# roseDwayane/EyeGaze-Multimodal

Measured on AMD Instinct MI355X. Metric: train samples/sec (gaze+EEG windows), higher is better.
Workload: dtype bf16; 1 GPU; cfg3: BASELINE configs[2]/[3]: + bidirectional cross-stream attention fusion; batch_per_gpu=256, global_batch=256, C=8, T=1024, seq_len=65, d_model=256, layers=6, step=fwd(train,dropout)+bwd+allreduce+clip+AdamW, parallelism=dp1

## Files before the change

### eyegaze_multimodal_amd/csrc/ffn.hip

```cpp
#include <type_traits>
#include "lnproj.h"

namespace {

constexpr int FR = RT_ROWS;
constexpr int FD = RT_COLS;
constexpr int FC = 128;
constexpr int F_XT = RT_TILEB;
constexpr int F_HT = FR * FC * 2;
constexpr int F_LDS = F_XT + 2 * F_HT;

template <typename T>
struct FfnArgs {
  const T* A; const T* W1; const T* W2; T* H; T* C; const float* bias1; const float* bias2; const T* gate; const T* residual;
  const unsigned long long* bits_in; unsigned long long* bits_out;
  const float* ln_gamma; const float* ln_beta; T* LN_OUT; float* ln_stats;
  const eg_step_state* st;
  long long lda, ldh, ldc, ldg, ldr;
  int M, F, relu, res_in_lds;
  DropCfg dh, dc1, dc2;
  float gate_scale;
};

struct FfnNoTail {};
template <typename T, int GATE, int BOUT, int EPI, bool LNF = false, bool KEEP = true, bool TAIL = false>
__global__ __launch_bounds__(256, 2) void ffn_chain_kernel(FfnArgs<T> p, std::conditional_t<TAIL, LnProjArgs<T>, FfnNoTail> q) {
  static_assert(!TAIL || (GATE == 2 && BOUT == 0 && EPI == 0 && !LNF && KEEP), "the norm-1 tail follows the backward form only");
  typedef typename H16<T>::frag frag;
  extern __shared__ __attribute__((aligned(16))) char smem[];
  char* const xt = smem;
  char* const hb = smem + F_XT;
  const int tid = threadIdx.x, lane = tid & 63;
  const int wn = __builtin_amdgcn_readfirstlane(tid >> 6);
  const int l15 = lane & 15, g4 = lane >> 4;
  const int m0 = blockIdx.x * FR;
  const int nch = p.F / FC;

#pragma unroll
  for (int i = 0; i < RT_DMA_PER_WAVE; ++i) {
    const int row = min(m0 + rt_dma_row(wn, lane, i), p.M - 1);
    rt_dma_issue((const char*)(p.A + (size_t)row * (size_t)p.lda), xt, wn, lane, i);
  }

  const char* const w1u = (const char*)(p.W1 + rt_frag_elem<8, 2>(0, wn, 0, 0));
  const char* const w2u = (const char*)(p.W2 + rt_frag_elem<4, 4>(0, wn, 0, 0));
  const uint32_t wl = (uint32_t)lane * 16u;
  frag w1r[4][2], w2r[2][4];
  auto req_w1 = [&](int c, int s, int slot) {
#pragma unroll
    for (int j = 0; j < 2; ++j) w1r[slot][j] = *(const frag*)(w1u + rt_frag_elem<8, 2>(c, 0, s, j) * 2 + wl);
  };
  auto req_w2 = [&](int c, int s, int slot) {
#pragma unroll
    for (int j = 0; j < 4; ++j) w2r[slot][j] = *(const frag*)(w2u + rt_frag_elem<4, 4>(c, 0, s, j) * 2 + wl);
  };
#pragma unroll
  for (int s = 0; s < 4; ++s) req_w1(0, s, s);
#pragma unroll
  for (int s = 0; s < 2; ++s) req_w2(0, s, s);

  f32x4 acc2[5][4];
#pragma unroll
  for (int i = 0; i < 5; ++i)
#pragma unroll
    for (int j = 0; j < 4; ++j) acc2[i][j] = (f32x4){0.f, 0.f, 0.f, 0.f};

  uint32_t seed_lo = 0, seed_hi = 0;
  if (p.dh.thresh | p.dc1.thresh | p.dc2.thresh) { seed_lo = p.st->seed_lo; seed_hi = p.st->seed_hi; }

  uint32_t touched = 0;
  if (wn < 2) {
    const char* wb = (const char*)(wn == 0 ? p.W1 : p.W2);
    const int lines = p.F * FD * 2 / 128;
    const int per = (lines + gridDim.x - 1) / gridDim.x;
    for (int t = lane; t < per; t += 64) {
      const int g = blockIdx.x * per + t;
      if (g < lines) touched += *(const uint32_t*)(wb + (size_t)g * 128);
    }
  }
  asm volatile("s_waitcnt vmcnt(0)" ::: "memory");
  asm volatile("" :: "v"(touched));
  __syncthreads();

  const unsigned long long* const bits_p = p.bits_in ? p.bits_in + ((size_t)blockIdx.x * nch * 4 + wn) * 64 + lane : nullptr;
  unsigned long long gnext0 = 0, gnext1 = 0;
  if (GATE == 2) {
    gnext0 = bits_p[0];
    if (nch > 1) gnext1 = bits_p[256];
  }
  const int rbase = l15;
  const int sw7 = rt_swz(l15);
  int ha[2];
#pragma unroll
  for (int j = 0; j < 2; ++j) {
    const int hcol = 32 * wn + 16 * j + 4 * g4;
    ha[j] = l15 * 256 + (((hcol >> 3) ^ sw7) << 4) + ((hcol & 4) << 1);
  }
  const uint32_t pair0 = ((uint32_t)(m0 + l15) * (uint32_t)p.F + (uint32_t)(32 * wn + 4 * g4)) >> 1;
  const uint32_t pairF = 8u * (uint32_t)p.F;

  for (int c = 0; c < nch; ++c) {
    char* const hc = hb + (c & 1) * F_HT;
    const int f0 = FC * c + 32 * wn + 4 * g4;

    float b1[2][4];
#pragma unroll
    for (int j = 0; j < 2; ++j) {
#pragma unroll
      for (int q = 0; q < 4; ++q) b1[j][q] = 0.f;
      if (EPI == 3 || (EPI == 4 && p.bias1)) load4(p.bias1 + f0 + 16 * j, b1[j]);
    }

    u32x2 gt[5][2];
    if (GATE == 1) {
      int rb = rbase;
      asm volatile("" : "+v"(rb));
#pragma unroll
      for (int i = 0; i < 5; ++i) {
        const int m = min(m0 + rb + 16 * i, p.M - 1);
#pragma unroll
        for (int j = 0; j < 2; ++j) gt[i][j] = *(const u32x2*)(p.gate + (size_t)m * (size_t)p.ldg + f0 + 16 * j);
      }
    }
    uint32_t gw[2] = {0u, 0u}, ow[2] = {0u, 0u};
    if (GATE == 2) {
      gw[0] = (uint32_t)gnext0;
      gw[1] = (uint32_t)(gnext0 >> 32);
      gnext0 = gnext1;
      if (c + 2 < nch) gnext1 = bits_p[(size_t)(c + 2) * 256];
    }

    f32x4 acc1[5][2];
#pragma unroll
    for (int i = 0; i < 5; ++i)
#pragma unroll
      for (int j = 0; j < 2; ++j) acc1[i][j] = (f32x4){0.f, 0.f, 0.f, 0.f};
#pragma unroll
    for (int s = 0; s < 8; ++s) {
      frag xf[5];
      rt_frags<T>(xt, rbase, g4, sw7, s, xf);
#pragma unroll
      for (int i = 0; i < 5; ++i)
#pragma unroll
        for (int j = 0; j < 2; ++j) acc1[i][j] = H16<T>::mfma(w1r[s & 3][j], xf[i], acc1[i][j]);
      if (s < 4) req_w1(c, s + 4, s & 3);
      else if (c + 1 < nch) req_w1(c + 1, s - 4, s & 3);
    }

    const uint32_t pairc = pair0 + (uint32_t)(FC / 2) * (uint32_t)c;
#pragma unroll
    for (int i = 0; i < 5; ++i) {
#pragma unroll
      for (int j = 0; j < 2; ++j) {
        const int t = 2 * i + j;
        float v[4];
#pragma unroll
        for (int q = 0; q < 4; ++q) {
          v[q] = acc1[i][j][q];
          if (EPI == 3 || EPI == 4) v[q] += b1[j][q];
          if (EPI == 3) v[q] = fmaxf(v[q], 0.f);
          if (EPI == 4 && p.relu) v[q] = fmaxf(v[q], 0.f);
        }
        if (GATE == 1) {
          float gv[4];
          load4((const T*)&gt[i][j], gv);
#pragma unroll
          for (int q = 0; q < 4; ++q) v[q] = gv[q] > 0.f ? v[q] * p.gate_scale : 0.f;
        }
        if (GATE == 2) {
#pragma unroll
          for (int q = 0; q < 4; ++q) {
            const int n = (2 * t + (q >> 1)) % 10;
            int m;
            asm("v_bfe_i32 %0, %1, %2, 1" : "=v"(m) : "v"(gw[t / 5]), "n"((9 - n) + 16 * (q & 1)));
            v[q] = __uint_as_float(__float_as_uint(v[q] * p.gate_scale) & (uint32_t)m);
          }
        }
        if (p.dh.thresh) {
          const uint32_t e = pairc + (uint32_t)(8 * j) + (uint32_t)i * pairF;
          const uint32_t h0 = eg_hash(seed_lo, seed_hi, p.dh.site, e), h1 = eg_hash(seed_lo, seed_hi, p.dh.site, e + 1u);
          v[0] = (h0 & 0xFFFFu) >= p.dh.thresh ? v[0] * p.dh.scale : 0.0f;
          v[1] = (h0 >> 16) >= p.dh.thresh ? v[1] * p.dh.scale : 0.0f;
          v[2] = (h1 & 0xFFFFu) >= p.dh.thresh ? v[2] * p.dh.scale : 0.0f;
          v[3] = (h1 >> 16) >= p.dh.thresh ? v[3] * p.dh.scale : 0.0f;
        }
        const u32x2 pk = pack4<T>(v);
        *(u32x2*)(hc + ha[j] + 4096 * i) = pk;
        if (BOUT) {
#pragma unroll
          for (int h = 0; h < 2; ++h) {
            uint32_t z, f;
            asm("v_pk_max_i16 %0, %1, 0" : "=v"(z) : "v"(pk[h]));
            asm("v_pk_min_u16 %0, %1, %2" : "=v"(f) : "v"(z), "v"(0x00010001u));
            ow[t / 5] = (ow[t / 5] << 1) | f;
          }
        }
      }
    }
    if (BOUT) p.bits_out[((size_t)blockIdx.x * nch + c) * 256 + wn * 64 + lane] = (unsigned long long)ow[0] | ((unsigned long long)ow[1] << 32);
    __syncthreads();

    if constexpr (KEEP) {
      int tq = tid >> 4;
      asm volatile("" : "+v"(tq));
#pragma unroll
      for (int ps = 0; ps < 5; ++ps) {
        const int r = 16 * ps + tq, ch = tid & 15;
        const u32x4 o = *(const u32x4*)(hc + r * 256 + rt_piece(r, ch));
        if (m0 + r < p.M) *(u32x4*)(p.H + (size_t)(m0 + r) * (size_t)p.ldh + FC * c + 8 * ch) = o;
      }
    }

#pragma unroll
    for (int s = 0; s < 4; ++s) {
      frag hf[5];
      rt_frags<T, FC * 2>(hc, rbase, g4, sw7, s, hf);
#pragma unroll
      for (int i = 0; i < 5; ++i)
#pragma unroll
        for (int j = 0; j < 4; ++j) acc2[i][j] = H16<T>::mfma(w2r[s & 1][j], hf[i], acc2[i][j]);
      if (s < 2) req_w2(c, s + 2, s & 1);
      else if (c + 1 < nch) req_w2(c + 1, s - 2, s & 1);
    }
  }
  __syncthreads();

  float* timg = (float*)(hb + wn * RT_IMGB);
  const int er = lane >> 2, ec = lane & 3;
  const int n = 64 * wn + 16 * ec;
  float bv[16];
#pragma unroll
  for (int j = 0; j < 16; ++j) bv[j] = 0.f;
  if (p.bias2) { load8(p.bias2 + n, bv); load8(p.bias2 + n + 8, bv + 8); }
  u32x4 eraw[5][2];
#pragma unroll
  for (int i = 0; i < 5; ++i) {
    eraw[i][0] = (u32x4){0u, 0u, 0u, 0u};
    eraw[i][1] = (u32x4){0u, 0u, 0u, 0u};
    const int r = 16 * i + er;
    if (p.res_in_lds) {
      rt_tile_row16(xt, r, n, eraw[i][0], eraw[i][1]);
    } else if (p.residual && m0 + r < p.M) {
      const T* pe = p.residual + (size_t)(m0 + r) * (size_t)p.ldr + n;
      eraw[i][0] = *(const u32x4*)pe;
      eraw[i][1] = *(const u32x4*)(pe + 8);
    }
  }
  const int tl = lane & 31, thw = tid >> 5;
  u32x4 xr[TAIL ? LP_ROWS_PER_HW : 1];
  float mean[TAIL ? LP_ROWS_PER_HW : 1], rstd[TAIL ? LP_ROWS_PER_HW : 1];
  if constexpr (TAIL) {
#pragma unroll
    for (int j = 0; j < LP_ROWS_PER_HW; ++j) {
      const int m = min(m0 + thw + 8 * j, q.M - 1);
      xr[j] = *(const u32x4*)(q.x + (size_t)m * FD + tl * 8);
    }
    lp_stats(q.stats, q.M, m0, thw, mean, rstd);
  }
  float vv[LNF ? 5 : 1][16];
  if (LNF) {
#pragma unroll
    for (int i = 0; i < 5; ++i)
#pragma unroll
      for (int j = 0; j < 16; ++j) vv[i][j] = 0.f;
  }
#pragma unroll
  for (int i = 0; i < 5; ++i) {
    const int m = m0 + 16 * i + er;
    rt_image_put(timg, acc2[i], lane);
    if (m0 + 16 * i >= p.M) break;
    float v[16];
    rt_image_get(timg, lane, v);
    if constexpr (TAIL) {
      if (m < p.M) {
        rt_row_epilogue<T, false, false>(v, bv, p.dc1, p.dc2, seed_lo, seed_hi, (uint32_t)m * (uint32_t)FD + (uint32_t)n,
                                         p.residual != nullptr, eraw[i][0], eraw[i][1], (T*)nullptr, vv[0]);
        if (p.C) rt_store16(p.C + (size_t)m * (size_t)p.ldc + n, v);
        const int r = 16 * i + er;
        store8((T*)(xt + r * RT_ROWB + rt_piece(r, n >> 3)), v);
        store8((T*)(xt + r * RT_ROWB + rt_piece(r, (n >> 3) + 1)), v + 8);
      }
    } else if (m < p.M)
      rt_row_epilogue<T, LNF, KEEP>(v, bv, p.dc1, p.dc2, seed_lo, seed_hi, (uint32_t)m * (uint32_t)FD + (uint32_t)n, p.residual != nullptr,
                                    eraw[i][0], eraw[i][1], KEEP ? p.C + (size_t)m * (size_t)p.ldc + n : nullptr, vv[LNF ? i : 0]);
  }
  if constexpr (TAIL) {
    const char* const wu = (const char*)(q.Wf + rt_frag_elem<4, 4>(0, wn, 0, 0));
    frag wr[2][4];
    float g[8], dg[8], db[8];
    load8(q.gamma + tl * 8, g);
#pragma unroll
    for (int e = 0; e < 8; ++e) { dg[e] = 0.f; db[e] = 0.f; }
    const bool drop = (q.d1.thresh | q.d2.thresh) != 0;
    uint32_t qs_lo = 0, qs_hi = 0;
    if (drop) { qs_lo = q.st->seed_lo; qs_hi = q.st->seed_hi; }
    lp_req_w<T>(wu, wl, 0, wr[0]);
    lp_req_w<T>(wu, wl, 1, wr[1]);
    __syncthreads();
    lp_ln_rows<T, true>(q, xt, nullptr, xr, m0, thw, tl, g, mean, rstd, drop, qs_lo, qs_hi, dg, db);
    __syncthreads();
    lp_sums(q.partial, (float*)hb, dg, db, tid, thw, tl);
    lp_product<T>(q.dC, q.M, xt, wr, wu, wl, (float*)(hb + LP_SUMS_B + wn * RT_IMGB), m0, lane, wn);
  }
  if constexpr (LNF)
    eg_epilogue_layernorm256<T>(vv, (float*)(hb + 4 * RT_IMGB), wn, lane, min(FR, p.M - m0), (size_t)m0, p.ln_gamma, p.ln_beta,
                                p.LN_OUT, KEEP ? p.ln_stats : nullptr);
}

template <typename T>
static FfnArgs<T> ffn_make_args(const eg_ffn_desc* d) {
  FfnArgs<T> p;
  p.A = (const T*)d->A; p.W1 = (const T*)d->W1; p.W2 = (const T*)d->W2; p.H = (T*)d->H; p.C = (T*)d->C;
  p.bits_in = (const unsigned long long*)d->gate_bits_in; p.bits_out = (unsigned long long*)d->gate_bits_out;
  p.bias1 = d->bias1; p.bias2 = d->bias2; p.gate = (const T*)d->gate; p.residual = (const T*)d->residual; p.st = d->state;
  p.lda = d->lda; p.ldh = d->ldh; p.ldc = d->ldc; p.ldg = d->ldg; p.ldr = d->ldr;
  p.M = d->M; p.F = d->F;
  p.relu = d->act1 == EG_ACT_RELU;
  p.res_in_lds = d->residual && d->residual == d->A && d->ldr == d->lda;
  p.dh = make_drop(d->drop_h_p, d->drop_h_site);
  p.dc1 = make_drop(d->drop_c1_p, d->drop_c1_site);
  p.dc2 = make_drop(d->drop_c2_p, d->drop_c2_site);
  p.gate_scale = d->gate_scale == 0.f ? 1.0f : d->gate_scale;
  p.ln_gamma = d->ln_gamma; p.ln_beta = d->ln_beta; p.LN_OUT = (T*)d->ln_out; p.ln_stats = d->ln_stats;
  return p;
}

template <typename T>
static int ffn_launch(const eg_ffn_desc* d, hipStream_t s) {
  const FfnArgs<T> p = ffn_make_args<T>(d);
  const FfnNoTail nt;
  const dim3 grid((d->M + FR - 1) / FR);
#define FFN_LAUNCH(G_, B_, E_, L_) eg_launch_lds<ffn_chain_kernel<T, G_, B_, E_, L_>, F_LDS>(grid, dim3(256), s, p, nt)
  const int gsel = d->gate_bits_in ? 2 : d->gate ? 1 : 0;
  const bool bout = d->gate_bits_out != nullptr;
  const bool lnf = d->ln_out != nullptr;
  if (!d->H) eg_launch_lds<ffn_chain_kernel<T, 0, 0, 3, true, false>, F_LDS>(grid, dim3(256), s, p, nt);
  else if (gsel == 0 && d->bias1 && p.relu) {
    if (lnf) { if (bout) FFN_LAUNCH(0, 1, 3, true); else FFN_LAUNCH(0, 0, 3, true); }
    else { if (bout) FFN_LAUNCH(0, 1, 3, false); else FFN_LAUNCH(0, 0, 3, false); }
  }
  else if (gsel == 2 && !d->bias1 && !p.relu) FFN_LAUNCH(2, 0, 0, false);
  else if (gsel == 1 && !d->bias1 && !p.relu) FFN_LAUNCH(1, 0, 0, false);
  else if (gsel == 2) FFN_LAUNCH(2, 0, 4, false);
  else if (gsel == 1) FFN_LAUNCH(1, 0, 4, false);
  else if (bout) FFN_LAUNCH(0, 1, 4, false);
  else FFN_LAUNCH(0, 0, 4, false);
#undef FFN_LAUNCH
  EG_LAUNCH_CHECK("ffn_chain");
  return 0;
}

template <typename T>
static int ffn_tail_launch(const eg_ffn_desc* f, const eg_ln_bwd_proj_desc* n, hipStream_t s) {
  const FfnArgs<T> p = ffn_make_args<T>(f);
  const LnProjArgs<T> q = lp_make_args<T>(n);
  eg_launch_lds<ffn_chain_kernel<T, 2, 0, 0, false, true, true>, F_LDS>(dim3((f->M + FR - 1) / FR), dim3(256), s, p, q);
  EG_LAUNCH_CHECK("ffn_bwd_ln_proj");
  return 0;
}

static int ffn_check_desc(const eg_ffn_desc* d, const char* who, bool tail) {
  EG_CHECK(d && d->A && d->W1 && d->W2, "%s: null operand", who);
  EG_CHECK(d->dtype == EG_BF16 || d->dtype == EG_F16, "%s: 16-bit compute dtypes only (got %d)", who, d->dtype);
  const bool lean = !tail && !d->H && !d->C;
  EG_CHECK(tail || lean || (d->H && d->C), "%s: H and C are both given (the keeping form) or both null (the lean form); got %s only", who,
           d->H ? "H" : "C");
  EG_CHECK(!lean || (d->bias1 && d->act1 == EG_ACT_RELU && !d->gate && !d->gate_bits_in),
           "%s: the lean form (H and C null) serves the forward form only: bias1, ReLU, no gate, no gate_bits_in", who);
  EG_CHECK(!lean || d->ln_out, "%s: the lean form (H and C null) needs ln_out, its only result", who);
  EG_CHECK(!lean || !d->gate_bits_out, "%s: the lean form (H and C null) writes no gate_bits_out", who);
  EG_CHECK(d->M > 0 && d->F > 0 && d->F % FC == 0, "%s: M=%d, F=%d (F must be a multiple of %d)", who, d->M, d->F, FC);
  EG_CHECK(d->act1 == EG_ACT_NONE || d->act1 == EG_ACT_RELU, "%s: act1 %d", who, d->act1);
  EG_CHECK(d->lda >= FD && d->lda % 8 == 0 && (lean || (d->ldh >= d->F && d->ldh % 8 == 0 && (!d->C || (d->ldc >= FD && d->ldc % 8 == 0)))),
           "%s: row strides must be 16-B multiples covering the rows", who);
  EG_CHECK(!d->gate || (d->ldg >= d->F && d->ldg % 4 == 0), "%s: gate stride", who);
  EG_CHECK(!(d->gate_bits_out && (d->gate_bits_in || d->gate)), "%s: a launch either writes gate bits or applies a gate", who);
  EG_CHECK(((uintptr_t)d->gate_bits_in | (uintptr_t)d->gate_bits_out) % 8 == 0, "%s: gate bit words must be 8-B aligned", who);
  EG_CHECK(!d->residual || (d->ldr >= FD && d->ldr % 8 == 0), "%s: residual stride", who);
  EG_CHECK((long long)d->M * d->F < (1ll << 32), "%s: M*F exceeds the 32-bit dropout index", who);
  EG_CHECK(!d->ln_out || (d->ln_gamma && d->ln_beta && (lean || d->ldc == FD) &&!d->gate && !d->gate_bits_in && d->bias1 && d->act1 == EG_ACT_RELU &&
                          (uintptr_t)d->ln_out % 16 == 0),
           "%s: the fused LayerNorm serves the forward form (bias + ReLU, no gate) with contiguous C rows", who);
  const float ps[3] = {d->drop_h_p, d->drop_c1_p, d->drop_c2_p};
  for (float q : ps) EG_CHECK(q >= 0.f && q < 1.f, "%s: dropout p", who);
  EG_CHECK((ps[0] == 0.f && ps[1] == 0.f && ps[2] == 0.f) || d->state, "%s: dropout needs a step state", who);
  EG_CHECK(((uintptr_t)d->A | (uintptr_t)d->W1 | (uintptr_t)d->W2 | (uintptr_t)d->H | (uintptr_t)d->C | (uintptr_t)d->gate |
            (uintptr_t)d->residual) % 16 == 0, "%s: operands must be 16-B aligned", who);
  return 0;
}

}

extern "C" int eg_ffn_chain(const eg_ffn_desc* d, void* stream) {
  if (int rc = ffn_check_desc(d, "eg_ffn_chain", false)) return rc;
  hipStream_t s = (hipStream_t)stream;
  return eg_dispatch_16(d->dtype, [&](auto t) { return ffn_launch<typename decltype(t)::type>(d, s); });
}

extern "C" int eg_ffn_bwd_ln_proj(const eg_ffn_desc* f, const eg_ln_bwd_proj_desc* n, void* stream) {
  static const char who[] = "eg_ffn_bwd_ln_proj";
  EG_CHECK(f && n, "%s: null descriptor", who);
  if (int rc = ffn_check_desc(f, who, true)) return rc;
  if (int rc = lp_check_desc(n, who, false)) return rc;
  EG_CHECK(f->gate_bits_in, "%s: f must be the backward form: gate_bits_in is not set", who);
  EG_CHECK(!f->bias1 && f->act1 == EG_ACT_NONE && !f->gate && !f->gate_bits_out && !f->ln_out,
           "%s: f must be the backward form: no bias1, act1, gate, gate_bits_out or ln_out", who);
  EG_CHECK(f->H, "%s: f->H (the hidden gradient rows) must be given; only f->C may be NULL", who);
  EG_CHECK(!n->dy || n->dy == f->C, "%s: n->dy must be NULL or f->C (the LayerNorm reads the rows the launch itself completes)", who);
  EG_CHECK(n->M == f->M, "%s: n->M=%d differs from f->M=%d", who, n->M, f->M);
  EG_CHECK(n->dtype == f->dtype, "%s: n->dtype=%d differs from f->dtype=%d", who, n->dtype, f->dtype);
  hipStream_t s = (hipStream_t)stream;
  return eg_dispatch_16(f->dtype, [&](auto t) { return ffn_tail_launch<typename decltype(t)::type>(f, n, s); });
}

extern "C" int64_t eg_ffn_gate_bits_bytes(int M, int F) {
  if (M <= 0 || F <= 0) return 0;
  return (int64_t)((M + FR - 1) / FR) * (F / FC) * 256 * 8;
}
```

Measured before the change: 86920 samples/s.

## Software-pipeline FFN chunks: overlap epilogue-1 of chunk c with GEMM-2 of c-1

Restructures the FFN chain loop so that the first GEMM's epilogue for chunk c (bias, ReLU, gate, dropout, pack to LDS) is interleaved with the second GEMM's MFMAs on chunk c-1's hidden tile. sched_group_barrier pins are used to mix VALU and MFMA work. When the hidden tile is kept, its global store is spread across the first-GEMM steps instead of running after the barrier. Dropout becomes a compile-time template flag so kernels without dropout drop the hash code. This adds code size, register pressure and scheduling fragility, and the double-buffered hidden tile now carries a one-chunk lag.

Result: faster. 88260 samples/s (median of 6 runs) (+1.5%).

```diff
diff --git a/eyegaze_multimodal_amd/csrc/ffn.hip b/eyegaze_multimodal_amd/csrc/ffn.hip
--- a/eyegaze_multimodal_amd/csrc/ffn.hip
+++ b/eyegaze_multimodal_amd/csrc/ffn.hip
@@ -9,6 +9,16 @@
 constexpr int F_XT = RT_TILEB;
 constexpr int F_HT = FR * FC * 2;
 constexpr int F_LDS = F_XT + 2 * F_HT;
+
+template <int LEAD, int PER>
+__device__ __forceinline__ void ffn_pin() {
+  __builtin_amdgcn_sched_group_barrier(0x2, LEAD, 0);
+#pragma unroll
+  for (int g = 0; g < 8; ++g) {
+    __builtin_amdgcn_sched_group_barrier(0x8, 1, 0);
+    __builtin_amdgcn_sched_group_barrier(0x2, PER, 0);
+  }
+}
 
 template <typename T>
 struct FfnArgs {
@@ -23,7 +33,7 @@
 };
 
 struct FfnNoTail {};
-template <typename T, int GATE, int BOUT, int EPI, bool LNF = false, bool KEEP = true, bool TAIL = false>
+template <typename T, int GATE, int BOUT, int EPI, bool LNF = false, bool KEEP = true, bool TAIL = false, bool DROP = false>
 __global__ __launch_bounds__(256, 2) void ffn_chain_kernel(FfnArgs<T> p, std::conditional_t<TAIL, LnProjArgs<T>, FfnNoTail> q) {
   static_assert(!TAIL || (GATE == 2 && BOUT == 0 && EPI == 0 && !LNF && KEEP), "the norm-1 tail follows the backward form only");
   typedef typename H16<T>::frag frag;
@@ -35,6 +45,7 @@
   const int l15 = lane & 15, g4 = lane >> 4;
   const int m0 = blockIdx.x * FR;
   const int nch = p.F / FC;
+  constexpr bool SPREAD = KEEP && EPI != 4 && GATE != 1;
 
 #pragma unroll
   for (int i = 0; i < RT_DMA_PER_WAVE; ++i) {
@@ -56,8 +67,6 @@
   };
 #pragma unroll
   for (int s = 0; s < 4; ++s) req_w1(0, s, s);
-#pragma unroll
-  for (int s = 0; s < 2; ++s) req_w2(0, s, s);
 
   f32x4 acc2[5][4];
 #pragma unroll
@@ -89,29 +98,32 @@
     if (nch > 1) gnext1 = bits_p[256];
   }
   const int rbase = l15;
-  const int sw7 = rt_swz(l15);
-  int ha[2];
-#pragma unroll
-  for (int j = 0; j < 2; ++j) {
-    const int hcol = 32 * wn + 16 * j + 4 * g4;
-    ha[j] = l15 * 256 + (((hcol >> 3) ^ sw7) << 4) + ((hcol & 4) << 1);
-  }
-  const uint32_t pair0 = ((uint32_t)(m0 + l15) * (uint32_t)p.F + (uint32_t)(32 * wn + 4 * g4)) >> 1;
+  struct E1Lane { int ha[2]; uint32_t pairc; };
+  auto e1_lane = [&](int c, int l15o, int g4o) __attribute__((always_inline)) {
+    E1Lane e;
+#pragma unroll
+    for (int j = 0; j < 2; ++j) {
+      const int hcol = 32 * wn + 16 * j + 4 * g4o;
+      e.ha[j] = l15o * 256 + (((hcol >> 3) ^ rt_swz(l15o)) << 4) + ((hcol & 4) << 1);
+    }
+    e.pairc = (((uint32_t)(m0 + l15o) * (uint32_t)p.F + (uint32_t)(32 * wn + 4 * g4o)) >> 1) + (uint32_t)(FC / 2) * (uint32_t)c;
+    return e;
+  };
   const uint32_t pairF = 8u * (uint32_t)p.F;
 
-  for (int c = 0; c < nch; ++c) {
-    char* const hc = hb + (c & 1) * F_HT;
+  f32x4 acc1[5][2];
+  float b1[2][4];
+  u32x2 gt[5][2];
+  uint32_t gw[2] = {0u, 0u};
+
+  auto req_e1 = [&](int c) __attribute__((always_inline)) {
     const int f0 = FC * c + 32 * wn + 4 * g4;
-
-    float b1[2][4];
 #pragma unroll
     for (int j = 0; j < 2; ++j) {
 #pragma unroll
       for (int q = 0; q < 4; ++q) b1[j][q] = 0.f;
       if (EPI == 3 || (EPI == 4 && p.bias1)) load4(p.bias1 + f0 + 16 * j, b1[j]);
     }
-
-    u32x2 gt[5][2];
     if (GATE == 1) {
       int rb = rbase;
       asm volatile("" : "+v"(rb));
@@ -122,85 +134,134 @@
         for (int j = 0; j < 2; ++j) gt[i][j] = *(const u32x2*)(p.gate + (size_t)m * (size_t)p.ldg + f0 + 16 * j);
       }
     }
-    uint32_t gw[2] = {0u, 0u}, ow[2] = {0u, 0u};
     if (GATE == 2) {
       gw[0] = (uint32_t)gnext0;
       gw[1] = (uint32_t)(gnext0 >> 32);
       gnext0 = gnext1;
       if (c + 2 < nch) gnext1 = bits_p[(size_t)(c + 2) * 256];
     }
-
-    f32x4 acc1[5][2];
+  };
+
+  auto product1 = [&](int c, int cst = -1) __attribute__((always_inline)) {
 #pragma unroll
     for (int i = 0; i < 5; ++i)
 #pragma unroll
       for (int j = 0; j < 2; ++j) acc1[i][j] = (f32x4){0.f, 0.f, 0.f, 0.f};
+    int lo = lane;
+    asm volatile("" : "+v"(lo));
+    const int l15o = lo & 15, g4o = lo >> 4, sw7o = rt_swz(l15o);
 #pragma unroll
     for (int s = 0; s < 8; ++s) {
       frag xf[5];
-      rt_frags<T>(xt, rbase, g4, sw7, s, xf);
+      rt_frags<T>(xt, l15o, g4o, sw7o, s, xf);
 #pragma unroll
       for (int i = 0; i < 5; ++i)
 #pragma unroll
         for (int j = 0; j < 2; ++j) acc1[i][j] = H16<T>::mfma(w1r[s & 3][j], xf[i], acc1[i][j]);
       if (s < 4) req_w1(c, s + 4, s & 3);
       else if (c + 1 < nch) req_w1(c + 1, s - 4, s & 3);
-    }
-
-    const uint32_t pairc = pair0 + (uint32_t)(FC / 2) * (uint32_t)c;
-#pragma unroll
-    for (int i = 0; i < 5; ++i) {
-#pragma unroll
-      for (int j = 0; j < 2; ++j) {
-        const int t = 2 * i + j;
-        float v[4];
-#pragma unroll
-        for (int q = 0; q < 4; ++q) {
-          v[q] = acc1[i][j][q];
-          if (EPI == 3 || EPI == 4) v[q] += b1[j][q];
-          if (EPI == 3) v[q] = fmaxf(v[q], 0.f);
-          if (EPI == 4 && p.relu) v[q] = fmaxf(v[q], 0.f);
+      if (SPREAD && cst >= 0 && s >= 1 && s <= 5) {
+        const int ps = s - 1, r = 16 * ps + (tid >> 4), ch = tid & 15;
+        const u32x4 o = *(const u32x4*)(hb + (cst & 1) * F_HT + r * 256 + rt_piece(r, ch));
+        if (m0 + r < p.M) *(u32x4*)(p.H + (size_t)(m0 + r) * (size_t)p.ldh + FC * cst + 8 * ch) = o;
+      }
+    }
+  };
+
+  auto p2_frag = [&](const char* hc, int g, int l15o, int g4o) __attribute__((always_inline)) {
+    return *(const frag*)(hc + (l15o + 16 * (g % 5)) * (FC * 2) + (((4 * (g / 5) + g4o) ^ rt_swz(l15o)) << 4));
+  };
+  auto p2_group = [&](int g, const frag& hf) __attribute__((always_inline)) {
+#pragma unroll
+    for (int j = 0; j < 4; ++j) acc2[g % 5][j] = H16<T>::mfma(w2r[(g / 5) & 1][j], hf, acc2[g % 5][j]);
+  };
+
+  auto e1_tile = [&](int t, char* hc, const E1Lane& el, uint32_t (&ow)[2]) __attribute__((always_inline)) {
+    const int i = t >> 1, j = t & 1;
+    float v[4];
+#pragma unroll
+    for (int q = 0; q < 4; ++q) {
+      v[q] = acc1[i][j][q];
+      if (EPI == 3 || EPI == 4) v[q] += b1[j][q];
+      if (EPI == 3) v[q] = fmaxf(v[q], 0.f);
+      if (EPI == 4 && p.relu) v[q] = fmaxf(v[q], 0.f);
+    }
+    if (GATE == 1) {
+      float gv[4];
+      load4((const T*)&gt[i][j], gv);
+#pragma unroll
+      for (int q = 0; q < 4; ++q) v[q] = gv[q] > 0.f ? v[q] * p.gate_scale : 0.f;
+    }
+    if (GATE == 2) {
+#pragma unroll
+      for (int q = 0; q < 4; ++q) {
+        const int n = (2 * t + (q >> 1)) % 10;
+        int m;
+        asm("v_bfe_i32 %0, %1, %2, 1" : "=v"(m) : "v"(gw[t / 5]), "n"((9 - n) + 16 * (q & 1)));
+        v[q] = __uint_as_float(__float_as_uint(v[q] * p.gate_scale) & (uint32_t)m);
+      }
+    }
+    if (DROP) {
+      const uint32_t e = el.pairc + (uint32_t)(8 * j) + (uint32_t)i * pairF;
+      const uint32_t h0 = eg_hash(seed_lo, seed_hi, p.dh.site, e), h1 = eg_hash(seed_lo, seed_hi, p.dh.site, e + 1u);
+      v[0] = (h0 & 0xFFFFu) >= p.dh.thresh ? v[0] * p.dh.scale : 0.0f;
+      v[1] = (h0 >> 16) >= p.dh.thresh ? v[1] * p.dh.scale : 0.0f;
+      v[2] = (h1 & 0xFFFFu) >= p.dh.thresh ? v[2] * p.dh.scale : 0.0f;
+      v[3] = (h1 >> 16) >= p.dh.thresh ? v[3] * p.dh.scale : 0.0f;
+    }
+    const u32x2 pk = pack4<T>(v);
+    *(u32x2*)(hc + el.ha[j] + 4096 * i) = pk;
+    if (BOUT) {
+#pragma unroll
+      for (int h = 0; h < 2; ++h) {
+        uint32_t z, f;
+        asm("v_pk_max_i16 %0, %1, 0" : "=v"(z) : "v"(pk[h]));
+        asm("v_pk_min_u16 %0, %1, %2" : "=v"(f) : "v"(z), "v"(0x00010001u));
+        ow[t / 5] = (ow[t / 5] << 1) | f;
+      }
+    }
+  };
+
+  auto merged = [&](int c, uint32_t (&ow)[2]) __attribute__((always_inline)) {
+    char* const hc = hb + (c & 1) * F_HT;
+    const char* const hp = hb + ((c & 1) ^ 1) * F_HT;
+    int lo = lane;
+    asm volatile("" : "+v"(lo));
+    const int l15o = lo & 15, g4o = lo >> 4;
+    const E1Lane el = e1_lane(c, l15o, g4o);
+#pragma unroll
+    for (int t = 0; t < 10; ++t) {
+      const frag hf0 = p2_frag(hp, 2 * t, l15o, g4o), hf1 = p2_frag(hp, 2 * t + 1, l15o, g4o);
+      e1_tile(t, hc, el, ow);
+      p2_group(2 * t, hf0);
+      p2_group(2 * t + 1, hf1);
+#pragma unroll
+      for (int u = 0; u < 2; ++u)
+        if ((2 * t + u) % 5 == 4) {
+          const int s = (2 * t + u) / 5;
+          if (s < 2) req_w2(c - 1, s + 2, s & 1);
+          else req_w2(c, s - 2, s & 1);
         }
-        if (GATE == 1) {
-          float gv[4];
-          load4((const T*)&gt[i][j], gv);
-#pragma unroll
-          for (int q = 0; q < 4; ++q) v[q] = gv[q] > 0.f ? v[q] * p.gate_scale : 0.f;
-        }
-        if (GATE == 2) {
-#pragma unroll
-          for (int q = 0; q < 4; ++q) {
-            const int n = (2 * t + (q >> 1)) % 10;
-            int m;
-            asm("v_bfe_i32 %0, %1, %2, 1" : "=v"(m) : "v"(gw[t / 5]), "n"((9 - n) + 16 * (q & 1)));
-            v[q] = __uint_as_float(__float_as_uint(v[q] * p.gate_scale) & (uint32_t)m);
-          }
-        }
-        if (p.dh.thresh) {
-          const uint32_t e = pairc + (uint32_t)(8 * j) + (uint32_t)i * pairF;
-          const uint32_t h0 = eg_hash(seed_lo, seed_hi, p.dh.site, e), h1 = eg_hash(seed_lo, seed_hi, p.dh.site, e + 1u);
-          v[0] = (h0 & 0xFFFFu) >= p.dh.thresh ? v[0] * p.dh.scale : 0.0f;
-          v[1] = (h0 >> 16) >= p.dh.thresh ? v[1] * p.dh.scale : 0.0f;
-          v[2] = (h1 & 0xFFFFu) >= p.dh.thresh ? v[2] * p.dh.scale : 0.0f;
-          v[3] = (h1 >> 16) >= p.dh.thresh ? v[3] * p.dh.scale : 0.0f;
-        }
-        const u32x2 pk = pack4<T>(v);
-        *(u32x2*)(hc + ha[j] + 4096 * i) = pk;
-        if (BOUT) {
-#pragma unroll
-          for (int h = 0; h < 2; ++h) {
-            uint32_t z, f;
-            asm("v_pk_max_i16 %0, %1, 0" : "=v"(z) : "v"(pk[h]));
-            asm("v_pk_min_u16 %0, %1, %2" : "=v"(f) : "v"(z), "v"(0x00010001u));
-            ow[t / 5] = (ow[t / 5] << 1) | f;
-          }
-        }
-      }
-    }
+      if (DROP) ffn_pin<16, 8>();
+      else ffn_pin<2, 2>();
+      __builtin_amdgcn_sched_barrier(0);
+    }
+  };
+  auto e1_alone = [&](uint32_t (&ow)[2]) __attribute__((always_inline)) {
+    int lo = lane;
+    asm volatile("" : "+v"(lo));
+    const E1Lane el = e1_lane(0, lo & 15, lo >> 4);
+#pragma unroll
+    for (int t = 0; t < 10; ++t) {
+      e1_tile(t, hb, el, ow);
+      __builtin_amdgcn_sched_barrier(0);
+    }
+  };
+  auto publish = [&](int c, const uint32_t (&ow)[2], bool store = true) __attribute__((always_inline)) {
+    const char* const hc = hb + (c & 1) * F_HT;
     if (BOUT) p.bits_out[((size_t)blockIdx.x * nch + c) * 256 + wn * 64 + lane] = (unsigned long long)ow[0] | ((unsigned long long)ow[1] << 32);
     __syncthreads();
-
-    if constexpr (KEEP) {
+    if (KEEP && store) {
       int tq = tid >> 4;
       asm volatile("" : "+v"(tq));
 #pragma unroll
@@ -210,18 +271,37 @@
         if (m0 + r < p.M) *(u32x4*)(p.H + (size_t)(m0 + r) * (size_t)p.ldh + FC * c + 8 * ch) = o;
       }
     }
-
+  };
+
+  {
+    uint32_t ow[2] = {0u, 0u};
+    req_e1(0);
+    product1(0);
+    e1_alone(ow);
+#pragma unroll
+    for (int s = 0; s < 2; ++s) req_w2(0, s, s);
+    for (int c = 1; c < nch; ++c) {
+      publish(c - 1, ow, !SPREAD);
+      ow[0] = 0u; ow[1] = 0u;
+      req_e1(c);
+      product1(c, SPREAD ? c - 1 : -1);
+      merged(c, ow);
+    }
+    publish(nch - 1, ow);
+    const char* const hp = hb + ((nch - 1) & 1) * F_HT;
+    int lo = lane;
+    asm volatile("" : "+v"(lo));
+    const int l15o = lo & 15, g4o = lo >> 4;
 #pragma unroll
     for (int s = 0; s < 4; ++s) {
       frag hf[5];
-      rt_frags<T, FC * 2>(hc, rbase, g4, sw7, s, hf);
-#pragma unroll
-      for (int i = 0; i < 5; ++i)
-#pragma unroll
-        for (int j = 0; j < 4; ++j) acc2[i][j] = H16<T>::mfma(w2r[s & 1][j], hf[i], acc2[i][j]);
-      if (s < 2) req_w2(c, s + 2, s & 1);
-      else if (c + 1 < nch) req_w2(c + 1, s - 2, s & 1);
-    }
+#pragma unroll
+      for (int i = 0; i < 5; ++i) hf[i] = p2_frag(hp, 5 * s + i, l15o, g4o);
+#pragma unroll
+      for (int i = 0; i < 5; ++i) p2_group(5 * s + i, hf[i]);
+      if (s < 2) req_w2(nch - 1, s + 2, s & 1);
+    }
+    __builtin_amdgcn_sched_barrier(0);
   }
   __syncthreads();
 
@@ -330,11 +410,16 @@
   const FfnArgs<T> p = ffn_make_args<T>(d);
   const FfnNoTail nt;
   const dim3 grid((d->M + FR - 1) / FR);
-#define FFN_LAUNCH(G_, B_, E_, L_) eg_launch_lds<ffn_chain_kernel<T, G_, B_, E_, L_>, F_LDS>(grid, dim3(256), s, p, nt)
+#define FFN_LAUNCH_K(G_, B_, E_, L_, K_, T_, Q_)                                                                  \
+  do {                                                                                                            \
+    if (p.dh.thresh) eg_launch_lds<ffn_chain_kernel<T, G_, B_, E_, L_, K_, T_, true>, F_LDS>(grid, dim3(256), s, p, Q_);  \
+    else eg_launch_lds<ffn_chain_kernel<T, G_, B_, E_, L_, K_, T_, false>, F_LDS>(grid, dim3(256), s, p, Q_);             \
+  } while (0)
+#define FFN_LAUNCH(G_, B_, E_, L_) FFN_LAUNCH_K(G_, B_, E_, L_, true, false, nt)
   const int gsel = d->gate_bits_in ? 2 : d->gate ? 1 : 0;
   const bool bout = d->gate_bits_out != nullptr;
   const bool lnf = d->ln_out != nullptr;
-  if (!d->H) eg_launch_lds<ffn_chain_kernel<T, 0, 0, 3, true, false>, F_LDS>(grid, dim3(256), s, p, nt);
+  if (!d->H) FFN_LAUNCH_K(0, 0, 3, true, false, false, nt);
   else if (gsel == 0 && d->bias1 && p.relu) {
     if (lnf) { if (bout) FFN_LAUNCH(0, 1, 3, true); else FFN_LAUNCH(0, 0, 3, true); }
     else { if (bout) FFN_LAUNCH(0, 1, 3, false); else FFN_LAUNCH(0, 0, 3, false); }
@@ -345,7 +430,6 @@
   else if (gsel == 1) FFN_LAUNCH(1, 0, 4, false);
   else if (bout) FFN_LAUNCH(0, 1, 4, false);
   else FFN_LAUNCH(0, 0, 4, false);
-#undef FFN_LAUNCH
   EG_LAUNCH_CHECK("ffn_chain");
   return 0;
 }
@@ -354,7 +438,10 @@
 static int ffn_tail_launch(const eg_ffn_desc* f, const eg_ln_bwd_proj_desc* n, hipStream_t s) {
   const FfnArgs<T> p = ffn_make_args<T>(f);
   const LnProjArgs<T> q = lp_make_args<T>(n);
-  eg_launch_lds<ffn_chain_kernel<T, 2, 0, 0, false, true, true>, F_LDS>(dim3((f->M + FR - 1) / FR), dim3(256), s, p, q);
+  const dim3 grid((f->M + FR - 1) / FR);
+  FFN_LAUNCH_K(2, 0, 0, false, true, true, q);
+#undef FFN_LAUNCH
+#undef FFN_LAUNCH_K
   EG_LAUNCH_CHECK("ffn_bwd_ln_proj");
   return 0;
 }
```
